# kan-bayashi/espnet

Measured on AMD Instinct MI355X. Metric: frames/sec, 12L Conformer hybrid CTC/attention training step (B=32 T=1000 d=256 per GPU), higher is better.
Workload: dtype f32; 1 GPU; BASELINE configs[1]: 12L Conformer enc d=256 h=4 ff=2048 k=31 macaron+cnn rel_pos, 6L Transformer dec, V=5000, fbank B=32 T=1000 L=100, mtlalpha 0.3, lsm 0.1; global_batch=32, frames=1000, parallelism=dp1, optimizer=adam+noam, clip 5.0, launch=hipGraph, wgrad_side_stream=False, optimizer_steps_done=113

## Files before the change

### espnet_amd/csrc/ffn_f32.hip

```cpp
#include <stdlib.h>
#include <type_traits>
#include "common.h"
#include "../../include/espnet_amd.h"
#include "ffn_ln.h"
#include "ln_bwd_rows.h"

bool eamd_ffn_bf16_ok(const eamd_ffn_t* p);
int eamd_ffn_bf16_launch(const eamd_ffn_t* p, int bwd, void* stream);

namespace {

constexpr int FBM = 32;
constexpr int FD = 256;
constexpr int FHC = 128;
constexpr int FNT = 512;
constexpr int XS_LD = 264;
constexpr int HS_LD = 136;
constexpr int XS_SZ = FBM * XS_LD;
constexpr int HS_SZ = FBM * HS_LD;

constexpr int D_SMEM_FLOATS = XS_SZ + 4 * HS_SZ;

template <bool BWD, int ACT>
__global__ __launch_bounds__(FNT, 2) void ffn_f32_direct_kernel(const eamd_ffn_t p) {
  extern __shared__ __attribute__((aligned(16))) float sm[];
  float* const xs = sm;
  float* const hs = xs + XS_SZ;
  float* const fs = hs + 2 * HS_SZ;
  const int t = threadIdx.x;
  const int lane = t & 63, wave = __builtin_amdgcn_readfirstlane(t >> 6);
  const bool up = wave < 4;
  const int wq = wave & 3;
  const int fr = lane & 15, fq = lane >> 4;
  const int m0 = blockIdx.x * FBM;
  const int F = p.F;
  const int nch = F / FHC / (int)gridDim.y;
  const int hid0 = (int)blockIdx.y * nch * FHC;
  const int nsteps = 8 * nch;
  const bool full_rows = m0 + FBM <= p.M;
  using T_ = std::true_type;
  using F_ = std::false_type;

  if (!BWD && p.ln_x) {
    ffn_ln_stage(p, m0, t, [&](int row, int col, float4 y) __attribute__((always_inline)) {
      *reinterpret_cast<f32x4*>(&xs[row * XS_LD + col]) = (f32x4){y.x, y.y, y.z, y.w};
    });
  } else {
#pragma unroll
    for (int i = 0; i < 4; ++i) {
      const int idx = t + FNT * i, row = idx >> 6, c4 = idx & 63;
      *reinterpret_cast<f32x4*>(&xs[row * XS_LD + c4 * 4]) =
          *reinterpret_cast<const f32x4*>(p.x + (long)min(m0 + row, p.M - 1) * FD + c4 * 4);
    }
  }
  __syncthreads();

  if (up) {
    const float* __restrict__ W = p.w1 + (long)hid0 * FD;
    const int lc0 = wq * 32 + 2 * fr;
    constexpr int LCJ = 1;
    f32x4 bs[4][4];
    f32x4 zacc[2][2], zold[2][2];
#pragma unroll
    for (int i = 0; i < 2; ++i)
#pragma unroll
      for (int j = 0; j < 2; ++j) { zacc[i][j] = (f32x4){0.f, 0.f, 0.f, 0.f}; zold[i][j] = zacc[i][j]; }
    const unsigned thr_in = eamd_drop_thr16(p.p_in);
    const float inv_in = p.p_in > 0.f ? eamd_drop_inv(thr_in) : 1.f;
    const unsigned seed_in = (!BWD && p.p_in > 0.f) ? eamd_drop_seed((const unsigned long long*)p.drop_step, p.salt_in) : 0u;
    float bpre[2] = {0.f, 0.f};
    float fpre[2][2][4];
    const unsigned e_toff = (unsigned)(((fq * 4) * F + lc0) * 4);

    auto load_b = [&](auto set_c, int g) __attribute__((always_inline)) {
      constexpr int SET = decltype(set_c)::value;
      const char* base = reinterpret_cast<const char*>(W) + ((long)min(g, nsteps - 1) * 4 + wq) * 4096 + lane * 16;
#pragma unroll
      for (int v = 0; v < 4; ++v) bs[SET][v] = *reinterpret_cast<const f32x4*>(base + v * 1024);
    };
    float fA[2][2][4];
    auto read_a = [&](auto s_c, auto half_c) __attribute__((always_inline)) {
      constexpr int s = decltype(s_c)::value, hh = decltype(half_c)::value;
#pragma unroll
      for (int i = 0; i < 2; ++i) {
        const float4 v = *reinterpret_cast<const float4*>(&xs[(i * 16 + fr) * XS_LD + s * 32 + hh * 16 + fq * 4]);
        fA[hh][i][0] = v.x; fA[hh][i][1] = v.y; fA[hh][i][2] = v.z; fA[hh][i][3] = v.w;
      }
    };
    auto mfma_half = [&](auto set_c, auto half_c) __attribute__((always_inline)) {
      constexpr int SET = decltype(set_c)::value, q = decltype(half_c)::value;
#pragma unroll
      for (int e = 0; e < 4; ++e)
#pragma unroll
        for (int i = 0; i < 2; ++i)
#pragma unroll
          for (int j = 0; j < 2; ++j) {
            const float b = BWD ? bs[SET][q * 2 + (e >> 1)][(e & 1) * 2 + j] : bs[SET][q * 2 + j][e];
            zacc[i][j] = __builtin_amdgcn_mfma_f32_16x16x4f32(fA[q][i][e], b, zacc[i][j], 0, 0, 0);
          }
    };
    auto epi_quarter = [&](auto i_c, auto rr_c, int c) __attribute__((always_inline)) {
      constexpr int i = decltype(i_c)::value, rr = decltype(rr_c)::value;
      float* hp = hs + (c & 1) * HS_SZ;
      float* fp = fs + (c & 1) * HS_SZ;
#pragma unroll
      for (int r2 = 0; r2 < 2; ++r2) {
        constexpr int dummy = 0; (void)dummy;
        const int r = rr * 2 + r2;
// ... 14 lines not shown
          for (int j = 0; j < 2; ++j) hv[j] = (zold[i][j][r] * fpre[i][j][r]) * p.alpha;
        }
        *reinterpret_cast<float2*>(&hp[(i * 16 + fq * 4 + r) * HS_LD + lc0]) = make_float2(hv[0], hv[1]);
      }
    };
    auto load_f = [&](int c) __attribute__((always_inline)) {
      const char* base = reinterpret_cast<const char*>(p.f + (long)m0 * F + hid0 + c * FHC);
#pragma unroll
      for (int i = 0; i < 2; ++i)
#pragma unroll
        for (int r = 0; r < 4; ++r) {
          const long ro = full_rows ? (long)(i * 16 + r) * F : (long)(min(m0 + i * 16 + fq * 4 + r, p.M - 1) - m0 - fq * 4) * F;
          const float2 v = *reinterpret_cast<const float2*>(base + ro * 4 + e_toff);
          fpre[i][0][r] = v.x; fpre[i][1][r] = v.y;
        }
    };
    auto step = [&](auto s_c, auto up_c, auto epi_c, int P) __attribute__((always_inline)) {
      constexpr int s = decltype(s_c)::value;
      constexpr bool UP = decltype(up_c)::value, EPI = decltype(epi_c)::value;
      if constexpr (UP) {
        load_b(std::integral_constant<int, (s + 3) & 3>{}, 8 * P + s + 3);
        if constexpr (s == 4) {
          if constexpr (BWD) load_f(P);
          else if (p.b1) { bpre[0] = p.b1[hid0 + P * FHC + lc0]; bpre[1] = p.b1[hid0 + P * FHC + lc0 + 1]; }
        }
        __builtin_amdgcn_sched_barrier(0);
        read_a(s_c, std::integral_constant<int, 1>{});
        mfma_half(std::integral_constant<int, s & 3>{}, std::integral_constant<int, 0>{});
      }
      if constexpr (EPI && s < 4) epi_quarter(std::integral_constant<int, s & 1>{}, std::integral_constant<int, (s / 2)>{}, P - 1);
      if constexpr (UP) {
        __builtin_amdgcn_sched_barrier(0);
        read_a(std::integral_constant<int, (s + 1) & 7>{}, std::integral_constant<int, 0>{});
        mfma_half(std::integral_constant<int, s & 3>{}, std::integral_constant<int, 1>{});
        if constexpr (s == 7) {
#pragma unroll
          for (int i = 0; i < 2; ++i)
#pragma unroll
            for (int j = 0; j < 2; ++j) { zold[i][j] = zacc[i][j]; zacc[i][j] = (f32x4){0.f, 0.f, 0.f, 0.f}; }
        }
      }
      if constexpr (s == 7) __syncthreads();
    };
    auto period = [&](auto up_c, auto epi_c, int P) __attribute__((always_inline)) {
      step(std::integral_constant<int, 0>{}, up_c, epi_c, P);
      step(std::integral_constant<int, 1>{}, up_c, epi_c, P);
      step(std::integral_constant<int, 2>{}, up_c, epi_c, P);
      step(std::integral_constant<int, 3>{}, up_c, epi_c, P);
      step(std::integral_constant<int, 4>{}, up_c, epi_c, P);
      step(std::integral_constant<int, 5>{}, up_c, epi_c, P);
      step(std::integral_constant<int, 6>{}, up_c, epi_c, P);
      step(std::integral_constant<int, 7>{}, up_c, epi_c, P);
    };
    load_b(std::integral_constant<int, 0>{}, 0);
    load_b(std::integral_constant<int, 1>{}, 1);
    load_b(std::integral_constant<int, 2>{}, 2);
    read_a(std::integral_constant<int, 0>{}, std::integral_constant<int, 0>{});
    period(T_{}, F_{}, 0);
    for (int P = 1; P < nch; ++P) period(T_{}, T_{}, P);
    period(F_{}, T_{}, nch);
    period(F_{}, F_{}, nch + 1);
  } else {
    const float* __restrict__ W = p.w2 + (long)hid0 * FD;
    f32x4 bs[4][4];
    f32x4 yacc[2][4];
#pragma unroll
    for (int i = 0; i < 2; ++i)
#pragma unroll
      for (int j = 0; j < 4; ++j) yacc[i][j] = (f32x4){0.f, 0.f, 0.f, 0.f};
    auto load_b = [&](auto set_c, int gd) __attribute__((always_inline)) {
      constexpr int SET = decltype(set_c)::value;
      const char* base = reinterpret_cast<const char*>(W) + ((long)min(max(gd, 0), nsteps - 1) * 4 + wq) * 4096 + lane * 16;
#pragma unroll
      for (int v = 0; v < 4; ++v) bs[SET][v] = *reinterpret_cast<const f32x4*>(base + v * 1024);
    };
    float fA[2][2][4];
    auto read_a = [&](auto par_c, int sd, int hbuf) __attribute__((always_inline)) {
      constexpr int PAR = decltype(par_c)::value;
      const float* hp = hs + hbuf * HS_SZ;
#pragma unroll
      for (int i = 0; i < 2; ++i) {
        const float4 v = *reinterpret_cast<const float4*>(&hp[(i * 16 + fr) * HS_LD + sd * 16 + fq * 4]);
        fA[PAR][i][0] = v.x; fA[PAR][i][1] = v.y; fA[PAR][i][2] = v.z; fA[PAR][i][3] = v.w;
      }
    };
    auto mfma_step = [&](auto set_c, auto par_c) __attribute__((always_inline)) {
      constexpr int SET = decltype(set_c)::value, PAR = decltype(par_c)::value;
#pragma unroll
      for (int e = 0; e < 4; ++e)
#pragma unroll
        for (int i = 0; i < 2; ++i)
#pragma unroll
          for (int j = 0; j < 4; ++j) {
            const float b = BWD ? bs[SET][e][j] : bs[SET][j][e];
            yacc[i][j] = __builtin_amdgcn_mfma_f32_16x16x4f32(fA[PAR][i][e], b, yacc[i][j], 0, 0, 0);
          }
    };
    auto step = [&](auto s_c, auto d_c, auto dn_c, int P) __attribute__((always_inline)) {
      constexpr int s = decltype(s_c)::value;
      constexpr bool D = decltype(d_c)::value, DN = decltype(dn_c)::value;
      const int gd = 8 * (P - 2) + s;
      if constexpr (s + 3 < 8 ? D : DN) load_b(std::integral_constant<int, (s + 3) & 3>{}, gd + 3);
      if constexpr (D && (s == 1 || s == 3)) {
        float* dstp = (s == 1) ? p.h : (BWD ? nullptr : p.f);
        if (dstp) {
          const float* src = (s == 1 ? hs : fs) + (P & 1) * HS_SZ;
          const int dt = t - 256;
#pragma unroll
          for (int k = 0; k < 4; ++k) {
            const int idx = dt + 256 * k, lr = idx >> 5, c4 = idx & 31;
            if (full_rows || m0 + lr < p.M)
              *reinterpret_cast<float4*>(dstp + (long)(m0 + lr) * F + hid0 + (P - 2) * FHC + c4 * 4) =
                  *reinterpret_cast<const float4*>(&src[lr * HS_LD + c4 * 4]);
          }
        }
      }
      if constexpr (D) {
        __builtin_amdgcn_sched_barrier(0);
        if constexpr (s < 7) read_a(std::integral_constant<int, (s + 1) & 1>{}, s + 1, P & 1);
        mfma_step(std::integral_constant<int, s & 3>{}, std::integral_constant<int, s & 1>{});
      }
      if constexpr (s == 7) {
        __syncthreads();
        if constexpr (DN) read_a(std::integral_constant<int, 0>{}, 0, (P + 1) & 1);
      }
    };
    auto period = [&](auto d_c, auto dn_c, int P) __attribute__((always_inline)) {
      step(std::integral_constant<int, 0>{}, d_c, dn_c, P);
      step(std::integral_constant<int, 1>{}, d_c, dn_c, P);
      step(std::integral_constant<int, 2>{}, d_c, dn_c, P);
      step(std::integral_constant<int, 3>{}, d_c, dn_c, P);
      step(std::integral_constant<int, 4>{}, d_c, dn_c, P);
      step(std::integral_constant<int, 5>{}, d_c, dn_c, P);
      step(std::integral_constant<int, 6>{}, d_c, dn_c, P);
      step(std::integral_constant<int, 7>{}, d_c, dn_c, P);
    };
    period(F_{}, F_{}, 0);
    period(F_{}, T_{}, 1);
    for (int P = 2; P <= nch; ++P) period(T_{}, T_{}, P);
    period(T_{}, F_{}, nch + 1);
#pragma unroll
    for (int i = 0; i < 2; ++i)
#pragma unroll
      for (int r = 0; r < 4; ++r) {
        if constexpr (BWD) {
          *reinterpret_cast<float4*>(&xs[(i * 16 + fq * 4 + r) * XS_LD + wq * 64 + 4 * fr]) =
              make_float4(yacc[i][0][r], yacc[i][1][r], yacc[i][2][r], yacc[i][3][r]);
        } else {
#pragma unroll
          for (int j = 0; j < 4; ++j) xs[(i * 16 + fq * 4 + r) * XS_LD + wq * 64 + j * 16 + fr] = yacc[i][j][r];
        }
      }
  }
  __syncthreads();
  if constexpr (BWD) {
    if (p.lnb_x) {
      const EamdLnbArgs la{p.lnb_x, p.lnb_gamma, p.lnb_mean, p.lnb_rstd, p.lnb_dres, p.lnb_ws, p.lnb_drop_out, p.lnb_drop_p,
                           (unsigned long long)p.lnb_drop_salt, p.drop_step, p.out, (long)FD, p.M};
      eamd_ln_bwd_rows32<XS_LD>(la, xs, hs, hs + FBM * FD, m0, t, (int)blockIdx.x);
      return;
    }
  }
  const unsigned thr_out = eamd_drop_thr16(p.p_out);
  const float inv_out = eamd_drop_inv(thr_out);
  const unsigned seed_out = (!BWD && p.p_out > 0.f) ? eamd_drop_seed((const unsigned long long*)p.drop_step, p.salt_out) : 0u;
#pragma unroll
  for (int i = 0; i < 4; ++i) {
    const int idx = t + FNT * i, lr = idx >> 6, c4 = idx & 63;
    const int row = m0 + lr;
    if (row >= p.M) continue;
    const float4 a4 = *reinterpret_cast<const float4*>(&xs[lr * XS_LD + c4 * 4]);
    float v[4] = {a4.x, a4.y, a4.z, a4.w};
    const long gi = (long)row * FD + c4 * 4;
    const bool first = blockIdx.y == 0;
    if constexpr (!BWD) {
      if (p.b2 && first) {
        const float4 b4 = *reinterpret_cast<const float4*>(p.b2 + c4 * 4);
        v[0] += b4.x; v[1] += b4.y; v[2] += b4.z; v[3] += b4.w;
      }
      if (p.p_out > 0.f) {
        bool keep[4];
        eamd_drop_keep4(seed_out, (unsigned long long)gi, thr_out, keep);
#pragma unroll
        for (int e = 0; e < 4; ++e) v[e] = keep[e] ? v[e] * inv_out : 0.f;
      }
      float4 r4 = make_float4(0.f, 0.f, 0.f, 0.f);
      if (p.R && first) r4 = *reinterpret_cast<const float4*>(p.R + gi);
      v[0] = v[0] * p.alpha + r4.x; v[1] = v[1] * p.alpha + r4.y; v[2] = v[2] * p.alpha + r4.z; v[3] = v[3] * p.alpha + r4.w;
    }
    if (gridDim.y > 1) {
#pragma unroll
      for (int e = 0; e < 4; ++e) atomicAdd(p.out + gi + e, v[e]);
    } else {
      *reinterpret_cast<float4*>(p.out + gi) = make_float4(v[0], v[1], v[2], v[3]);
    }
  }
}

__global__ __launch_bounds__(256) void ffn_pack_f32_kernel(const float* __restrict__ w1, const float* __restrict__ w2,
                                                           float* __restrict__ p0, float* __restrict__ p1,
                                                           float* __restrict__ p2, float* __restrict__ p3, int F) {
  const int which = blockIdx.y;
  const long piece = (long)blockIdx.x * 256 + threadIdx.x;
  const long npiece = (long)(F / FHC) * 8 * 4 * 4 * 64;
  if (piece >= npiece) return;
  const int lane = piece & 63, v = (piece >> 6) & 3, wq = (piece >> 8) & 3;
  const int g = (int)(piece >> 10), c = g >> 3, s = g & 7;
  const int fr = lane & 15, fq = lane >> 4;
  float4 o;
  if (which == 0) {
    const int q = v >> 1, j = v & 1;
    o = *reinterpret_cast<const float4*>(w1 + (long)(c * FHC + wq * 32 + 2 * fr + j) * FD + s * 32 + q * 16 + fq * 4);
    *reinterpret_cast<float4*>(p0 + piece * 4) = o;
  } else if (which == 1) {
    o = *reinterpret_cast<const float4*>(w2 + (long)(wq * 64 + v * 16 + fr) * F + c * FHC + s * 16 + fq * 4);
    *reinterpret_cast<float4*>(p1 + piece * 4) = o;
  } else if (which == 2) {
    const int q = v >> 1, e0 = (v & 1) * 2;
    const float* r0 = w2 + (long)(s * 32 + q * 16 + fq * 4 + e0) * F + c * FHC + wq * 32 + 2 * fr;
    const float2 a = *reinterpret_cast<const float2*>(r0), b = *reinterpret_cast<const float2*>(r0 + F);
    *reinterpret_cast<float4*>(p2 + piece * 4) = make_float4(a.x, a.y, b.x, b.y);
  } else {
    o = *reinterpret_cast<const float4*>(w1 + (long)(c * FHC + s * 16 + fq * 4 + v) * FD + wq * 64 + 4 * fr);
    *reinterpret_cast<float4*>(p3 + piece * 4) = o;
  }
}

constexpr int FFN_PACK_JOBS = 32;
struct FfnPackJob { const float* w1; const float* w2; float* p0; float* p1; float* p2; float* p3; int F; int pad; };
struct FfnPackTable { FfnPackJob j[FFN_PACK_JOBS]; };
__global__ __launch_bounds__(256) void ffn_pack_f32_multi_kernel(const FfnPackTable tab) {
  const FfnPackJob jb = tab.j[blockIdx.z];
  const int which = blockIdx.y, F = jb.F;
  const long npiece = (long)(F / FHC) * 8 * 4 * 4 * 64;
  for (long piece = (long)blockIdx.x * 256 + threadIdx.x; piece < npiece; piece += (long)gridDim.x * 256) {
    const int lane = piece & 63, v = (piece >> 6) & 3, wq = (piece >> 8) & 3;
    const int g = (int)(piece >> 10), c = g >> 3, s = g & 7;
    const int fr = lane & 15, fq = lane >> 4;
    if (which == 0) {
      const int q = v >> 1, j = v & 1;
// ... 126 lines not shown
```

### espnet_amd/csrc/ffn_ln.h

```cpp
#pragma once
#include "common.h"
#include "../../include/espnet_amd.h"

template <typename Put>
__device__ __forceinline__ void ffn_ln_stage(const eamd_ffn_t& p, const int m0, const int t, Put&& put) {
  constexpr int D = 256;
  const int row = t >> 4, l = t & 15;
  const bool live = m0 + row < p.M;
  const long gr = (long)min(m0 + row, p.M - 1);
  const float4* __restrict__ xr = reinterpret_cast<const float4*>(p.ln_x + gr * D);
  float4 v[4];
  float s = 0.f;
#pragma unroll
  for (int j = 0; j < 4; ++j) { v[j] = xr[l + 16 * j]; s += v[j].x + v[j].y + v[j].z + v[j].w; }
#pragma unroll
  for (int m = 1; m < 16; m <<= 1) s += __shfl_xor(s, m);
  const float mean = s / D;
  float q = 0.f;
#pragma unroll
  for (int j = 0; j < 4; ++j) {
    const float a = v[j].x - mean, b = v[j].y - mean, c = v[j].z - mean, d = v[j].w - mean;
    q += a * a + b * b + c * c + d * d;
  }
#pragma unroll
  for (int m = 1; m < 16; m <<= 1) q += __shfl_xor(q, m);
  const float rstd = rsqrtf(q / D + p.ln_eps);
  const float4* __restrict__ g4 = reinterpret_cast<const float4*>(p.ln_w);
  const float4* __restrict__ b4 = reinterpret_cast<const float4*>(p.ln_b);
#pragma unroll
  for (int j = 0; j < 4; ++j) {
    const float4 g = g4[l + 16 * j], b = b4[l + 16 * j];
    float4 o;
    o.x = (v[j].x - mean) * rstd * g.x + b.x;
    o.y = (v[j].y - mean) * rstd * g.y + b.y;
    o.z = (v[j].z - mean) * rstd * g.z + b.z;
    o.w = (v[j].w - mean) * rstd * g.w + b.w;
    const int col = (l + 16 * j) * 4;
    put(row, col, o);
    if (live) {
      if (p.dtype == 1) {
        uint2 h;
        h.x = eamd_f2bf(o.x) | ((unsigned)eamd_f2bf(o.y) << 16);
        h.y = eamd_f2bf(o.z) | ((unsigned)eamd_f2bf(o.w) << 16);
        *reinterpret_cast<uint2*>(reinterpret_cast<unsigned short*>(const_cast<float*>(p.x)) + gr * D + col) = h;
      } else {
        *reinterpret_cast<float4*>(const_cast<float*>(p.x) + gr * D + col) = o;
      }
    }
  }
  if (live && l == 0) { p.ln_mean[gr] = mean; p.ln_rstd[gr] = rstd; }
}
```

### espnet_amd/csrc/ln_bwd_rows.h

```cpp
#pragma once
#include "common.h"

struct EamdLnbArgs {
  const float* x; const float* gamma; const float* mean; const float* rstd; const float* dres;
  float* ws; float* drop_out; float drop_p; unsigned long long drop_salt; const void* drop_step;
  float* out; long ldo; int M;
};

template <int TLD>
__device__ __forceinline__ void eamd_ln_bwd_rows32(const EamdLnbArgs& a, const float* tile, float* gs, float* bsum, const int m0,
                                                   const int t, const int blk) {
  constexpr int D = 256;
  const int row = t >> 4, l = t & 15;
  const bool live = m0 + row < a.M;
  const long gr = (long)min(m0 + row, a.M - 1);
  const float mu = a.mean[gr], rs = a.rstd[gr];
  float4 dq[4], h4[4], g4[4], rv[4];
  float s1 = 0.f, s2 = 0.f;
#pragma unroll
  for (int j = 0; j < 4; ++j) {
    const int col = (l + 16 * j) * 4;
    dq[j] = *reinterpret_cast<const float4*>(&tile[row * TLD + col]);
    const float4 xv = *reinterpret_cast<const float4*>(a.x + gr * D + col);
    g4[j] = *reinterpret_cast<const float4*>(a.gamma + col);
    rv[j] = a.dres ? *reinterpret_cast<const float4*>(a.dres + gr * D + col) : make_float4(0.f, 0.f, 0.f, 0.f);
    h4[j] = make_float4((xv.x - mu) * rs, (xv.y - mu) * rs, (xv.z - mu) * rs, (xv.w - mu) * rs);
    const float p0 = dq[j].x * g4[j].x, p1 = dq[j].y * g4[j].y, p2 = dq[j].z * g4[j].z, p3 = dq[j].w * g4[j].w;
    s1 += (p0 + p1) + (p2 + p3);
    s2 += (p0 * h4[j].x + p1 * h4[j].y) + (p2 * h4[j].z + p3 * h4[j].w);
  }
#pragma unroll
  for (int m = 1; m < 16; m <<= 1) { s1 += __shfl_xor(s1, m); s2 += __shfl_xor(s2, m); }
  s1 /= D; s2 /= D;
  const unsigned thr_d = eamd_drop_thr16(a.drop_p);
  const float inv_d = eamd_drop_inv(thr_d);
  const unsigned seed_d = a.drop_out ? eamd_drop_seed((const unsigned long long*)a.drop_step, a.drop_salt) : 0u;
  const float z = live ? 1.f : 0.f;
#pragma unroll
  for (int j = 0; j < 4; ++j) {
    const int col = (l + 16 * j) * 4;
    float4 o;
    o.x = rs * (dq[j].x * g4[j].x - s1 - h4[j].x * s2) + rv[j].x;
    o.y = rs * (dq[j].y * g4[j].y - s1 - h4[j].y * s2) + rv[j].y;
    o.z = rs * (dq[j].z * g4[j].z - s1 - h4[j].z * s2) + rv[j].z;
    o.w = rs * (dq[j].w * g4[j].w - s1 - h4[j].w * s2) + rv[j].w;
    if (live) {
      *reinterpret_cast<float4*>(a.out + gr * a.ldo + col) = o;
      if (a.drop_out) {
        bool keep[4];
        eamd_drop_keep4(seed_d, (unsigned long long)(gr * D + col), thr_d, keep);
        *reinterpret_cast<float4*>(a.drop_out + gr * D + col) =
            make_float4(keep[0] ? o.x * inv_d : 0.f, keep[1] ? o.y * inv_d : 0.f, keep[2] ? o.z * inv_d : 0.f,
                        keep[3] ? o.w * inv_d : 0.f);
      }
    }
    *reinterpret_cast<float4*>(&gs[row * D + col]) =
        make_float4(z * dq[j].x * h4[j].x, z * dq[j].y * h4[j].y, z * dq[j].z * h4[j].z, z * dq[j].w * h4[j].w);
    *reinterpret_cast<float4*>(&bsum[row * D + col]) = make_float4(z * dq[j].x, z * dq[j].y, z * dq[j].z, z * dq[j].w);
  }
  __syncthreads();
  const float* src = (t < D ? gs : bsum) + (t & (D - 1));
  float s = 0.f;
#pragma unroll 8
  for (int r = 0; r < 32; ++r) s += src[r * D];
  a.ws[(long)blk * 2 * D + t] = s;
}
```

### espnet_amd/csrc/rowproj_f32.hip

```cpp
#include <stdlib.h>
#include <type_traits>
#include "common.h"
#include "../../include/espnet_amd.h"
#include "ln_bwd_rows.h"

namespace {

constexpr int RBM = 32;
constexpr int RNT = 512;
constexpr int RCH = 256;
constexpr int ST_LD = 36;
constexpr int ST_SZ = RBM * ST_LD;
constexpr int TL_LD = 264;

__device__ __forceinline__ int xs_ld(int K) { return K + 8; }

__device__ __forceinline__ void stage_ln(const eamd_rowproj_t& p, const int m0, const int t, float* xs, const int LD) {
  constexpr int D = 256;
  const int row = t >> 4, l = t & 15;
  const bool live = m0 + row < p.M;
  const long gr = (long)min(m0 + row, p.M - 1);
  const float4* __restrict__ xr = reinterpret_cast<const float4*>(p.ln_x + gr * D);
  float4 v[4];
  float s = 0.f;
#pragma unroll
  for (int j = 0; j < 4; ++j) { v[j] = xr[l + 16 * j]; s += v[j].x + v[j].y + v[j].z + v[j].w; }
#pragma unroll
  for (int m = 1; m < 16; m <<= 1) s += __shfl_xor(s, m);
  const float mean = s / D;
  float q = 0.f;
#pragma unroll
  for (int j = 0; j < 4; ++j) {
    const float a = v[j].x - mean, b = v[j].y - mean, c = v[j].z - mean, d = v[j].w - mean;
    q += a * a + b * b + c * c + d * d;
  }
#pragma unroll
  for (int m = 1; m < 16; m <<= 1) q += __shfl_xor(q, m);
  const float rstd = rsqrtf(q / D + p.ln_eps);
  const float4* __restrict__ g4 = reinterpret_cast<const float4*>(p.ln_w);
  const float4* __restrict__ b4 = reinterpret_cast<const float4*>(p.ln_b);
#pragma unroll
  for (int j = 0; j < 4; ++j) {
    const float4 g = g4[l + 16 * j], b = b4[l + 16 * j];
    float4 o;
    o.x = (v[j].x - mean) * rstd * g.x + b.x;
    o.y = (v[j].y - mean) * rstd * g.y + b.y;
    o.z = (v[j].z - mean) * rstd * g.z + b.z;
    o.w = (v[j].w - mean) * rstd * g.w + b.w;
    const int col = (l + 16 * j) * 4;
    *reinterpret_cast<float4*>(&xs[row * LD + col]) = o;
    if (live) *reinterpret_cast<float4*>(const_cast<float*>(p.a) + gr * D + col) = o;
  }
  if (live && l == 0) { p.ln_mean[gr] = mean; p.ln_rstd[gr] = rstd; }
}

__device__ __forceinline__ void stage_affine(const eamd_rowproj_t& p, const int m0, const int t, float* xs, const int LD) {
  constexpr int D = 256;
#pragma unroll
  for (int i = 0; i < 4; ++i) {
    const int idx = t + RNT * i, row = idx >> 6, c4 = idx & 63;
    const long gr = (long)min(m0 + row, p.M - 1);
    const float4 v = *reinterpret_cast<const float4*>(p.a + gr * p.lda + c4 * 4);
    const float4 sc = *reinterpret_cast<const float4*>(p.a_scale + c4 * 4), sh = *reinterpret_cast<const float4*>(p.a_shift + c4 * 4);
    float4 o;
    o.x = eamd_act(v.x * sc.x + sh.x, p.a_act); o.y = eamd_act(v.y * sc.y + sh.y, p.a_act);
    o.z = eamd_act(v.z * sc.z + sh.z, p.a_act); o.w = eamd_act(v.w * sc.w + sh.w, p.a_act);
    *reinterpret_cast<float4*>(&xs[row * LD + c4 * 4]) = o;
    if (p.a_out && m0 + row < p.M) *reinterpret_cast<float4*>(p.a_out + gr * D + c4 * 4) = o;
  }
}

template <bool LNB>
__global__ __launch_bounds__(RNT, 2) void rowproj_f32_kernel(const eamd_rowproj_t p) {
  extern __shared__ __attribute__((aligned(16))) float sm[];
  const int K = p.K, N = p.N;
  const int LD = xs_ld(K);
  float* const xs = sm;
  const int t = threadIdx.x;
  const int lane = t & 63, wave = __builtin_amdgcn_readfirstlane(t >> 6);
  const int fr = lane & 15, fq = lane >> 4;
  const int m0 = blockIdx.x * RBM;
  const int S = K >> 5;
  const int nchunk = N / RCH;
  const int nsteps = S * nchunk;
  float* const st = sm + RBM * LD + wave * ST_SZ;

  if (p.ln_x) {
    stage_ln(p, m0, t, xs, LD);
  } else if (p.a_scale) {
    stage_affine(p, m0, t, xs, LD);
  } else {
    const int c4n = K >> 2;
    for (int idx = t; idx < RBM * c4n; idx += RNT) {
      const int row = idx / c4n, c4 = idx - row * c4n;
      *reinterpret_cast<f32x4*>(&xs[row * LD + c4 * 4]) =
          *reinterpret_cast<const f32x4*>(p.a + (long)min(m0 + row, p.M - 1) * p.lda + c4 * 4);
    }
  }

  const char* __restrict__ Wb = reinterpret_cast<const char*>(p.w) + (long)wave * 4096 + lane * 16;
  f32x4 bs[4][4];
  auto load_b = [&](auto set_c, int g) __attribute__((always_inline)) {
    constexpr int SET = decltype(set_c)::value;
    const char* base = Wb + (long)min(g, nsteps - 1) * (8 * 4096);
#pragma unroll
    for (int v = 0; v < 4; ++v) bs[SET][v] = *reinterpret_cast<const f32x4*>(base + v * 1024);
  };
  float fA[2][2][4];
  auto read_a = [&](int kcol, auto half_c) __attribute__((always_inline)) {
    constexpr int hh = decltype(half_c)::value;
#pragma unroll
    for (int i = 0; i < 2; ++i) {
      const float4 v = *reinterpret_cast<const float4*>(&xs[(i * 16 + fr) * LD + kcol + hh * 16 + fq * 4]);
      fA[hh][i][0] = v.x; fA[hh][i][1] = v.y; fA[hh][i][2] = v.z; fA[hh][i][3] = v.w;
    }
  };
  f32x4 acc[2][2];
  auto mfma_half = [&](auto set_c, auto half_c) __attribute__((always_inline)) {
    constexpr int SET = decltype(set_c)::value, q = decltype(half_c)::value;
#pragma unroll
    for (int e = 0; e < 4; ++e)
#pragma unroll
      for (int i = 0; i < 2; ++i)
#pragma unroll
        for (int j = 0; j < 2; ++j)
          acc[i][j] = __builtin_amdgcn_mfma_f32_16x16x4f32(fA[q][i][e], bs[SET][q * 2 + j][e], acc[i][j], 0, 0, 0);
  };
  using I0 = std::integral_constant<int, 0>;
  using I1 = std::integral_constant<int, 1>;
  auto step = [&](auto s_c, int g, int kcol, int kcol_next) __attribute__((always_inline)) {
    constexpr int s = decltype(s_c)::value;
    load_b(std::integral_constant<int, (s + 3) & 3>{}, g + 3);
    __builtin_amdgcn_sched_barrier(0);
    read_a(kcol, I1{});
    mfma_half(std::integral_constant<int, s & 3>{}, I0{});
    __builtin_amdgcn_sched_barrier(0);
    read_a(kcol_next, I0{});
    mfma_half(std::integral_constant<int, s & 3>{}, I1{});
  };

  load_b(std::integral_constant<int, 0>{}, 0);
  load_b(std::integral_constant<int, 1>{}, 1);
  load_b(std::integral_constant<int, 2>{}, 2);
  __syncthreads();
  read_a(0, I0{});

  const unsigned thr_out = eamd_drop_thr16(p.p_out);
  const float inv_out = eamd_drop_inv(thr_out);
  const unsigned seed_out = p.p_out > 0.f ? eamd_drop_seed((const unsigned long long*)p.drop_step, p.salt_out) : 0u;

  int g = 0;
  for (int c = 0; c < nchunk; ++c) {
#pragma unroll
    for (int i = 0; i < 2; ++i)
#pragma unroll
      for (int j = 0; j < 2; ++j) acc[i][j] = (f32x4){0.f, 0.f, 0.f, 0.f};
    for (int kp = 0; kp < S; kp += 4) {
      const int k0 = kp * 32;
      step(std::integral_constant<int, 0>{}, g + 0, k0, k0 + 32);
      step(std::integral_constant<int, 1>{}, g + 1, k0 + 32, k0 + 64);
      step(std::integral_constant<int, 2>{}, g + 2, k0 + 64, k0 + 96);
      step(std::integral_constant<int, 3>{}, g + 3, k0 + 96, (kp + 4 < S) ? k0 + 128 : 0);
      g += 4;
    }
    if constexpr (!LNB) {
#pragma unroll
      for (int i = 0; i < 2; ++i)
#pragma unroll
        for (int r = 0; r < 4; ++r)
          *reinterpret_cast<float2*>(&st[(i * 16 + fq * 4 + r) * ST_LD + 2 * fr]) = make_float2(acc[i][0][r], acc[i][1][r]);
      __builtin_amdgcn_fence(__ATOMIC_RELEASE, "wavefront");
      __builtin_amdgcn_wave_barrier();
      __builtin_amdgcn_fence(__ATOMIC_ACQUIRE, "wavefront");
      const int col0 = c * RCH + wave * 32 + (lane & 7) * 4;
      float4 b4 = make_float4(0.f, 0.f, 0.f, 0.f);
      if (p.bias) b4 = *reinterpret_cast<const float4*>(p.bias + col0);
#pragma unroll
      for (int it = 0; it < 4; ++it) {
        const int lr = it * 8 + (lane >> 3);
        const int row = m0 + lr;
        const float4 a4 = *reinterpret_cast<const float4*>(&st[lr * ST_LD + (lane & 7) * 4]);
        if (row < p.M) {
          float v[4] = {a4.x + b4.x, a4.y + b4.y, a4.z + b4.z, a4.w + b4.w};
          const long gi = (long)row * N + col0;
          if (p.p_out > 0.f) {
            bool keep[4];
            eamd_drop_keep4(seed_out, (unsigned long long)gi, thr_out, keep);
#pragma unroll
            for (int e = 0; e < 4; ++e) v[e] = keep[e] ? v[e] * inv_out : 0.f;
          }
          float4 r4 = make_float4(0.f, 0.f, 0.f, 0.f);
          if (p.R) r4 = *reinterpret_cast<const float4*>(p.R + (long)row * p.ldr + col0);
          *reinterpret_cast<float4*>(p.out + (long)row * p.ldo + col0) =
              make_float4(v[0] * p.alpha + r4.x, v[1] * p.alpha + r4.y, v[2] * p.alpha + r4.z, v[3] * p.alpha + r4.w);
        }
      }
      __builtin_amdgcn_wave_barrier();
    }
  }

  if constexpr (LNB) {
    constexpr int D = 256;
    float* const tl = sm;
    float* const gs = sm + RBM * TL_LD;
    float* const bsum = gs + RBM * D;
    __syncthreads();
#pragma unroll
    for (int i = 0; i < 2; ++i)
#pragma unroll
      for (int r = 0; r < 4; ++r)
        *reinterpret_cast<float2*>(&tl[(i * 16 + fq * 4 + r) * TL_LD + wave * 32 + 2 * fr]) = make_float2(acc[i][0][r], acc[i][1][r]);
    __syncthreads();
    const EamdLnbArgs la{p.lnb_x, p.lnb_gamma, p.lnb_mean, p.lnb_rstd, p.lnb_dres, p.lnb_ws, p.lnb_drop_out, p.lnb_drop_p,
                         (unsigned long long)p.lnb_drop_salt, p.drop_step, p.out, (long)p.ldo, p.M};
    eamd_ln_bwd_rows32<TL_LD>(la, tl, gs, bsum, m0, t, (int)blockIdx.x);
  }
}

struct PackJob { const float* w; float* img; int K, N, ldw, trans; long npiece; };
constexpr int PACK_JOBS = 48;
struct PackTable { PackJob j[PACK_JOBS]; };
__global__ __launch_bounds__(256) void rowproj_pack_kernel(const PackTable tab) {
  const PackJob jb = tab.j[blockIdx.y];
  for (long piece = (long)blockIdx.x * 256 + threadIdx.x; piece < jb.npiece; piece += (long)gridDim.x * 256) {
    const int lane = piece & 63, v = (piece >> 6) & 3, w = (piece >> 8) & 7;
    const long gs_ = piece >> 11;
    const int S = jb.K >> 5;
    const int c = (int)(gs_ / S), s = (int)(gs_ - (long)c * S);
    const int fr = lane & 15, fq = lane >> 4, q = v >> 1, j = v & 1;
    const int col = c * RCH + w * 32 + 2 * fr + j, k = s * 32 + q * 16 + fq * 4;
    float4 o;
    if (jb.trans) {
      const float* r0 = jb.w + (long)k * jb.ldw + col;
      o = make_float4(r0[0], r0[jb.ldw], r0[2L * jb.ldw], r0[3L * jb.ldw]);
    } else {
      o = *reinterpret_cast<const float4*>(jb.w + (long)col * jb.ldw + k);
    }
    *reinterpret_cast<float4*>(jb.img + piece * 4) = o;
  }
}

bool al16(const void* q) { return (reinterpret_cast<uintptr_t>(q) & 15) == 0; }

size_t smem_bytes(int K, bool lnb) {
  size_t rows = (size_t)RBM * (K + 8);
  if (lnb) {
    const size_t need = (size_t)RBM * TL_LD + 2 * (size_t)RBM * 256;
    return (rows > need ? rows : need) * sizeof(float);
  }
  return (rows + 8 * (size_t)ST_SZ) * sizeof(float);
}

int check_rowproj(const eamd_rowproj_t* p) {
  if (!p || !p->a || !p->w || !p->out) return EAMD_EINVAL;
  if (p->M <= 0 || p->K <= 0 || p->N <= 0) return EAMD_EINVAL;
  if (p->K % 256 != 0 || p->N % RCH != 0 || p->K > 768) return EAMD_EUNSUPPORTED;
  if (p->lda < p->K || p->ldo < p->N || (p->R && p->ldr < p->N)) return EAMD_EINVAL;
  if (p->lda % 4 != 0 || p->ldo % 4 != 0 || (p->R && p->ldr % 4 != 0)) return EAMD_EUNSUPPORTED;
  if (!al16(p->a) || !al16(p->w) || !al16(p->out) || (p->R && !al16(p->R)) || (p->bias && !al16(p->bias))) return EAMD_EUNSUPPORTED;
  if (p->p_out < 0.f || p->p_out >= 1.f) return EAMD_EINVAL;
  if (p->p_out > 0.f && (!p->drop_step || p->ldo != p->N)) return EAMD_EINVAL;
  if (p->ln_x) {
    if (p->K != 256 || p->a_scale || !p->ln_w || !p->ln_b || !p->ln_mean || !p->ln_rstd || p->lda != 256) return EAMD_EINVAL;
    if (!al16(p->ln_x) || !al16(p->ln_w) || !al16(p->ln_b)) return EAMD_EUNSUPPORTED;
  }
  if (p->a_scale) {
    if (p->K != 256 || !p->a_shift) return EAMD_EINVAL;
    if (!al16(p->a_scale) || !al16(p->a_shift) || (p->a_out && !al16(p->a_out))) return EAMD_EUNSUPPORTED;
// ... 57 lines not shown
```

Baseline: 1.147 million frames/s.

## Prefetch epilogue operands and overlap weight loads with row staging in FFN/rowproj kernels

The first weight-tile loads are now issued while activation rows are being staged, whether through LN, affine or a plain copy, instead of after staging finishes. Epilogue operands (residual, bias, and the LN-backward x/dres/gamma/mean/rstd) are prefetched into registers during the last MFMA steps rather than loaded after the GEMM. The goal is to hide global-memory latency at kernel start and in the epilogue. In exchange it raises register pressure, which may hurt occupancy at launch_bounds(512,2), and the rowproj K-loop is restructured to peel its last group.

```diff
diff --git a/espnet_amd/csrc/ffn_f32.hip b/espnet_amd/csrc/ffn_f32.hip
--- a/espnet_amd/csrc/ffn_f32.hip
+++ b/espnet_amd/csrc/ffn_f32.hip
@@ -41,19 +41,56 @@
   using T_ = std::true_type;
   using F_ = std::false_type;
 
-  if (!BWD && p.ln_x) {
-    ffn_ln_stage(p, m0, t, [&](int row, int col, float4 y) __attribute__((always_inline)) {
-      *reinterpret_cast<f32x4*>(&xs[row * XS_LD + col]) = (f32x4){y.x, y.y, y.z, y.w};
-    });
-  } else {
-#pragma unroll
-    for (int i = 0; i < 4; ++i) {
-      const int idx = t + FNT * i, row = idx >> 6, c4 = idx & 63;
-      *reinterpret_cast<f32x4*>(&xs[row * XS_LD + c4 * 4]) =
-          *reinterpret_cast<const f32x4*>(p.x + (long)min(m0 + row, p.M - 1) * FD + c4 * 4);
-    }
-  }
-  __syncthreads();
+  auto stage_rows = [&](auto&& issue_w) __attribute__((always_inline)) {
+    if (!BWD && p.ln_x) {
+      ffn_ln_stage(p, m0, t, [&](int row, int col, float4 y) __attribute__((always_inline)) {
+        *reinterpret_cast<f32x4*>(&xs[row * XS_LD + col]) = (f32x4){y.x, y.y, y.z, y.w};
+      }, issue_w);
+    } else {
+      f32x4 v[4];
+#pragma unroll
+      for (int i = 0; i < 4; ++i) {
+        const int idx = t + FNT * i, row = idx >> 6, c4 = idx & 63;
+        v[i] = *reinterpret_cast<const f32x4*>(p.x + (long)min(m0 + row, p.M - 1) * FD + c4 * 4);
+      }
+      issue_w();
+#pragma unroll
+      for (int i = 0; i < 4; ++i) {
+        const int idx = t + FNT * i, row = idx >> 6, c4 = idx & 63;
+        *reinterpret_cast<f32x4*>(&xs[row * XS_LD + c4 * 4]) = v[i];
+      }
+    }
+    __syncthreads();
+  };
+
+  const bool first = blockIdx.y == 0;
+  const EamdLnbArgs la{p.lnb_x, p.lnb_gamma, p.lnb_mean, p.lnb_rstd, p.lnb_dres, p.lnb_ws, p.lnb_drop_out, p.lnb_drop_p,
+                       (unsigned long long)p.lnb_drop_salt, p.drop_step, p.out, (long)FD, p.M};
+  EamdLnbPre pre;
+  float4 b2p = make_float4(0.f, 0.f, 0.f, 0.f), rp[4];
+  auto epi_pre = [&](auto part_c) __attribute__((always_inline)) {
+    constexpr int part = decltype(part_c)::value;
+    if constexpr (BWD) {
+      if (p.lnb_x) {
+        if constexpr (part == 0) eamd_ln_bwd_prefetch_x(la, pre, m0, t);
+        if constexpr (part == 1) eamd_ln_bwd_prefetch_dres(la, pre, m0, t);
+        if constexpr (part == 2) eamd_ln_bwd_prefetch_gamma(la, pre, t);
+      }
+    } else {
+      if constexpr (part == 0) {
+#pragma unroll
+        for (int i = 0; i < 4; ++i) rp[i] = make_float4(0.f, 0.f, 0.f, 0.f);
+        if (p.R && first) {
+#pragma unroll
+          for (int i = 0; i < 4; ++i)
+            rp[i] = *reinterpret_cast<const float4*>(p.R + (long)min(m0 + ((t + FNT * i) >> 6), p.M - 1) * FD + (t & 63) * 4);
+        }
+      }
+      if constexpr (part == 1) {
+        if (p.b2 && first) b2p = *reinterpret_cast<const float4*>(p.b2 + (t & 63) * 4);
+      }
+    }
+  };
 
   if (up) {
     const float* __restrict__ W = p.w1 + (long)hid0 * FD;
@@ -174,13 +211,18 @@
       step(std::integral_constant<int, 6>{}, up_c, epi_c, P);
       step(std::integral_constant<int, 7>{}, up_c, epi_c, P);
     };
-    load_b(std::integral_constant<int, 0>{}, 0);
-    load_b(std::integral_constant<int, 1>{}, 1);
-    load_b(std::integral_constant<int, 2>{}, 2);
+    stage_rows([&]() __attribute__((always_inline)) {
+      load_b(std::integral_constant<int, 0>{}, 0);
+      load_b(std::integral_constant<int, 1>{}, 1);
+      load_b(std::integral_constant<int, 2>{}, 2);
+    });
     read_a(std::integral_constant<int, 0>{}, std::integral_constant<int, 0>{});
     period(T_{}, F_{}, 0);
     for (int P = 1; P < nch; ++P) period(T_{}, T_{}, P);
     period(F_{}, T_{}, nch);
+    epi_pre(std::integral_constant<int, 0>{});
+    epi_pre(std::integral_constant<int, 1>{});
+    epi_pre(std::integral_constant<int, 2>{});
     period(F_{}, F_{}, nch + 1);
   } else {
     const float* __restrict__ W = p.w2 + (long)hid0 * FD;
@@ -223,6 +265,7 @@
       constexpr bool D = decltype(d_c)::value, DN = decltype(dn_c)::value;
       const int gd = 8 * (P - 2) + s;
       if constexpr (s + 3 < 8 ? D : DN) load_b(std::integral_constant<int, (s + 3) & 3>{}, gd + 3);
+      if constexpr (D && !DN && s >= 5) epi_pre(std::integral_constant<int, s - 5>{});
       if constexpr (D && (s == 1 || s == 3)) {
         float* dstp = (s == 1) ? p.h : (BWD ? nullptr : p.f);
         if (dstp) {
@@ -257,6 +300,7 @@
       step(std::integral_constant<int, 6>{}, d_c, dn_c, P);
       step(std::integral_constant<int, 7>{}, d_c, dn_c, P);
     };
+    stage_rows([]() {});
     period(F_{}, F_{}, 0);
     period(F_{}, T_{}, 1);
     for (int P = 2; P <= nch; ++P) period(T_{}, T_{}, P);
@@ -277,9 +321,7 @@
   __syncthreads();
   if constexpr (BWD) {
     if (p.lnb_x) {
-      const EamdLnbArgs la{p.lnb_x, p.lnb_gamma, p.lnb_mean, p.lnb_rstd, p.lnb_dres, p.lnb_ws, p.lnb_drop_out, p.lnb_drop_p,
-                           (unsigned long long)p.lnb_drop_salt, p.drop_step, p.out, (long)FD, p.M};
-      eamd_ln_bwd_rows32<XS_LD>(la, xs, hs, hs + FBM * FD, m0, t, (int)blockIdx.x);
+      eamd_ln_bwd_rows32<XS_LD>(la, pre, xs, hs, hs + FBM * FD, m0, t, (int)blockIdx.x);
       return;
     }
   }
@@ -294,10 +336,9 @@
     const float4 a4 = *reinterpret_cast<const float4*>(&xs[lr * XS_LD + c4 * 4]);
     float v[4] = {a4.x, a4.y, a4.z, a4.w};
     const long gi = (long)row * FD + c4 * 4;
-    const bool first = blockIdx.y == 0;
     if constexpr (!BWD) {
       if (p.b2 && first) {
-        const float4 b4 = *reinterpret_cast<const float4*>(p.b2 + c4 * 4);
+        const float4 b4 = b2p;
         v[0] += b4.x; v[1] += b4.y; v[2] += b4.z; v[3] += b4.w;
       }
       if (p.p_out > 0.f) {
@@ -306,8 +347,7 @@
 #pragma unroll
         for (int e = 0; e < 4; ++e) v[e] = keep[e] ? v[e] * inv_out : 0.f;
       }
-      float4 r4 = make_float4(0.f, 0.f, 0.f, 0.f);
-      if (p.R && first) r4 = *reinterpret_cast<const float4*>(p.R + gi);
+      const float4 r4 = rp[i];
       v[0] = v[0] * p.alpha + r4.x; v[1] = v[1] * p.alpha + r4.y; v[2] = v[2] * p.alpha + r4.z; v[3] = v[3] * p.alpha + r4.w;
     }
     if (gridDim.y > 1) {
diff --git a/espnet_amd/csrc/ffn_ln.h b/espnet_amd/csrc/ffn_ln.h
--- a/espnet_amd/csrc/ffn_ln.h
+++ b/espnet_amd/csrc/ffn_ln.h
@@ -2,17 +2,24 @@
 #include "common.h"
 #include "../../include/espnet_amd.h"
 
-template <typename Put>
-__device__ __forceinline__ void ffn_ln_stage(const eamd_ffn_t& p, const int m0, const int t, Put&& put) {
+template <typename Put, typename Issue>
+__device__ __forceinline__ void ffn_ln_stage(const eamd_ffn_t& p, const int m0, const int t, Put&& put, Issue&& issue_w) {
   constexpr int D = 256;
   const int row = t >> 4, l = t & 15;
   const bool live = m0 + row < p.M;
   const long gr = (long)min(m0 + row, p.M - 1);
   const float4* __restrict__ xr = reinterpret_cast<const float4*>(p.ln_x + gr * D);
-  float4 v[4];
+  const float4* __restrict__ g4 = reinterpret_cast<const float4*>(p.ln_w);
+  const float4* __restrict__ b4 = reinterpret_cast<const float4*>(p.ln_b);
+  float4 v[4], gv[4], bv[4];
+#pragma unroll
+  for (int j = 0; j < 4; ++j) v[j] = xr[l + 16 * j];
+#pragma unroll
+  for (int j = 0; j < 4; ++j) { gv[j] = g4[l + 16 * j]; bv[j] = b4[l + 16 * j]; }
+  issue_w();
   float s = 0.f;
 #pragma unroll
-  for (int j = 0; j < 4; ++j) { v[j] = xr[l + 16 * j]; s += v[j].x + v[j].y + v[j].z + v[j].w; }
+  for (int j = 0; j < 4; ++j) s += v[j].x + v[j].y + v[j].z + v[j].w;
 #pragma unroll
   for (int m = 1; m < 16; m <<= 1) s += __shfl_xor(s, m);
   const float mean = s / D;
@@ -25,11 +32,9 @@
 #pragma unroll
   for (int m = 1; m < 16; m <<= 1) q += __shfl_xor(q, m);
   const float rstd = rsqrtf(q / D + p.ln_eps);
-  const float4* __restrict__ g4 = reinterpret_cast<const float4*>(p.ln_w);
-  const float4* __restrict__ b4 = reinterpret_cast<const float4*>(p.ln_b);
 #pragma unroll
   for (int j = 0; j < 4; ++j) {
-    const float4 g = g4[l + 16 * j], b = b4[l + 16 * j];
+    const float4 g = gv[j], b = bv[j];
     float4 o;
     o.x = (v[j].x - mean) * rstd * g.x + b.x;
     o.y = (v[j].y - mean) * rstd * g.y + b.y;
@@ -50,3 +55,8 @@
   }
   if (live && l == 0) { p.ln_mean[gr] = mean; p.ln_rstd[gr] = rstd; }
 }
+
+template <typename Put>
+__device__ __forceinline__ void ffn_ln_stage(const eamd_ffn_t& p, const int m0, const int t, Put&& put) {
+  ffn_ln_stage(p, m0, t, put, []() {});
+}
diff --git a/espnet_amd/csrc/ln_bwd_rows.h b/espnet_amd/csrc/ln_bwd_rows.h
--- a/espnet_amd/csrc/ln_bwd_rows.h
+++ b/espnet_amd/csrc/ln_bwd_rows.h
@@ -7,23 +7,47 @@
   float* out; long ldo; int M;
 };
 
+struct EamdLnbPre { float mu, rs; float4 xv[4], g4[4], rv[4]; };
+
+__device__ __forceinline__ void eamd_ln_bwd_prefetch_x(const EamdLnbArgs& a, EamdLnbPre& pre, const int m0, const int t) {
+  constexpr int D = 256;
+  const int row = t >> 4, l = t & 15;
+  const long gr = (long)min(m0 + row, a.M - 1);
+  pre.mu = a.mean[gr]; pre.rs = a.rstd[gr];
+#pragma unroll
+  for (int j = 0; j < 4; ++j) pre.xv[j] = *reinterpret_cast<const float4*>(a.x + gr * D + (l + 16 * j) * 4);
+}
+__device__ __forceinline__ void eamd_ln_bwd_prefetch_dres(const EamdLnbArgs& a, EamdLnbPre& pre, const int m0, const int t) {
+  constexpr int D = 256;
+  const int row = t >> 4, l = t & 15;
+  const long gr = (long)min(m0 + row, a.M - 1);
+#pragma unroll
+  for (int j = 0; j < 4; ++j)
+    pre.rv[j] = a.dres ? *reinterpret_cast<const float4*>(a.dres + gr * D + (l + 16 * j) * 4) : make_float4(0.f, 0.f, 0.f, 0.f);
+}
+__device__ __forceinline__ void eamd_ln_bwd_prefetch_gamma(const EamdLnbArgs& a, EamdLnbPre& pre, const int t) {
+  const int l = t & 15;
+#pragma unroll
+  for (int j = 0; j < 4; ++j) pre.g4[j] = *reinterpret_cast<const float4*>(a.gamma + (l + 16 * j) * 4);
+}
+
 template <int TLD>
-__device__ __forceinline__ void eamd_ln_bwd_rows32(const EamdLnbArgs& a, const float* tile, float* gs, float* bsum, const int m0,
-                                                   const int t, const int blk) {
+__device__ __forceinline__ void eamd_ln_bwd_rows32(const EamdLnbArgs& a, const EamdLnbPre& pre, const float* tile, float* gs,
+                                                   float* bsum, const int m0, const int t, const int blk) {
   constexpr int D = 256;
   const int row = t >> 4, l = t & 15;
   const bool live = m0 + row < a.M;
   const long gr = (long)min(m0 + row, a.M - 1);
-  const float mu = a.mean[gr], rs = a.rstd[gr];
+  const float mu = pre.mu, rs = pre.rs;
   float4 dq[4], h4[4], g4[4], rv[4];
   float s1 = 0.f, s2 = 0.f;
 #pragma unroll
   for (int j = 0; j < 4; ++j) {
     const int col = (l + 16 * j) * 4;
     dq[j] = *reinterpret_cast<const float4*>(&tile[row * TLD + col]);
-    const float4 xv = *reinterpret_cast<const float4*>(a.x + gr * D + col);
-    g4[j] = *reinterpret_cast<const float4*>(a.gamma + col);
-    rv[j] = a.dres ? *reinterpret_cast<const float4*>(a.dres + gr * D + col) : make_float4(0.f, 0.f, 0.f, 0.f);
+    const float4 xv = pre.xv[j];
+    g4[j] = pre.g4[j];
+    rv[j] = pre.rv[j];
     h4[j] = make_float4((xv.x - mu) * rs, (xv.y - mu) * rs, (xv.z - mu) * rs, (xv.w - mu) * rs);
     const float p0 = dq[j].x * g4[j].x, p1 = dq[j].y * g4[j].y, p2 = dq[j].z * g4[j].z, p3 = dq[j].w * g4[j].w;
     s1 += (p0 + p1) + (p2 + p3);
diff --git a/espnet_amd/csrc/rowproj_f32.hip b/espnet_amd/csrc/rowproj_f32.hip
--- a/espnet_amd/csrc/rowproj_f32.hip
+++ b/espnet_amd/csrc/rowproj_f32.hip
@@ -15,16 +15,24 @@
 
 __device__ __forceinline__ int xs_ld(int K) { return K + 8; }
 
-__device__ __forceinline__ void stage_ln(const eamd_rowproj_t& p, const int m0, const int t, float* xs, const int LD) {
+template <typename Issue>
+__device__ __forceinline__ void stage_ln(const eamd_rowproj_t& p, const int m0, const int t, float* xs, const int LD, Issue&& issue_w) {
   constexpr int D = 256;
   const int row = t >> 4, l = t & 15;
   const bool live = m0 + row < p.M;
   const long gr = (long)min(m0 + row, p.M - 1);
   const float4* __restrict__ xr = reinterpret_cast<const float4*>(p.ln_x + gr * D);
-  float4 v[4];
+  const float4* __restrict__ g4 = reinterpret_cast<const float4*>(p.ln_w);
+  const float4* __restrict__ b4 = reinterpret_cast<const float4*>(p.ln_b);
+  float4 v[4], gv[4], bv[4];
+#pragma unroll
+  for (int j = 0; j < 4; ++j) v[j] = xr[l + 16 * j];
+#pragma unroll
+  for (int j = 0; j < 4; ++j) { gv[j] = g4[l + 16 * j]; bv[j] = b4[l + 16 * j]; }
+  issue_w();
   float s = 0.f;
 #pragma unroll
-  for (int j = 0; j < 4; ++j) { v[j] = xr[l + 16 * j]; s += v[j].x + v[j].y + v[j].z + v[j].w; }
+  for (int j = 0; j < 4; ++j) s += v[j].x + v[j].y + v[j].z + v[j].w;
 #pragma unroll
   for (int m = 1; m < 16; m <<= 1) s += __shfl_xor(s, m);
   const float mean = s / D;
@@ -37,11 +45,9 @@
 #pragma unroll
   for (int m = 1; m < 16; m <<= 1) q += __shfl_xor(q, m);
   const float rstd = rsqrtf(q / D + p.ln_eps);
-  const float4* __restrict__ g4 = reinterpret_cast<const float4*>(p.ln_w);
-  const float4* __restrict__ b4 = reinterpret_cast<const float4*>(p.ln_b);
 #pragma unroll
   for (int j = 0; j < 4; ++j) {
-    const float4 g = g4[l + 16 * j], b = b4[l + 16 * j];
+    const float4 g = gv[j], b = bv[j];
     float4 o;
     o.x = (v[j].x - mean) * rstd * g.x + b.x;
     o.y = (v[j].y - mean) * rstd * g.y + b.y;
@@ -54,20 +60,54 @@
   if (live && l == 0) { p.ln_mean[gr] = mean; p.ln_rstd[gr] = rstd; }
 }
 
-__device__ __forceinline__ void stage_affine(const eamd_rowproj_t& p, const int m0, const int t, float* xs, const int LD) {
+template <typename Issue>
+__device__ __forceinline__ void stage_affine(const eamd_rowproj_t& p, const int m0, const int t, float* xs, const int LD,
+                                             Issue&& issue_w) {
   constexpr int D = 256;
+  const int c4 = t & 63;
+  float4 vv[4];
+#pragma unroll
+  for (int i = 0; i < 4; ++i)
+    vv[i] = *reinterpret_cast<const float4*>(p.a + (long)min(m0 + ((t + RNT * i) >> 6), p.M - 1) * p.lda + c4 * 4);
+  const float4 sc = *reinterpret_cast<const float4*>(p.a_scale + c4 * 4), sh = *reinterpret_cast<const float4*>(p.a_shift + c4 * 4);
+  issue_w();
 #pragma unroll
   for (int i = 0; i < 4; ++i) {
-    const int idx = t + RNT * i, row = idx >> 6, c4 = idx & 63;
+    const int row = (t + RNT * i) >> 6;
     const long gr = (long)min(m0 + row, p.M - 1);
-    const float4 v = *reinterpret_cast<const float4*>(p.a + gr * p.lda + c4 * 4);
-    const float4 sc = *reinterpret_cast<const float4*>(p.a_scale + c4 * 4), sh = *reinterpret_cast<const float4*>(p.a_shift + c4 * 4);
+    const float4 v = vv[i];
     float4 o;
     o.x = eamd_act(v.x * sc.x + sh.x, p.a_act); o.y = eamd_act(v.y * sc.y + sh.y, p.a_act);
     o.z = eamd_act(v.z * sc.z + sh.z, p.a_act); o.w = eamd_act(v.w * sc.w + sh.w, p.a_act);
     *reinterpret_cast<float4*>(&xs[row * LD + c4 * 4]) = o;
     if (p.a_out && m0 + row < p.M) *reinterpret_cast<float4*>(p.a_out + gr * D + c4 * 4) = o;
   }
+}
+
+template <typename Issue>
+__device__ __forceinline__ void stage_plain(const eamd_rowproj_t& p, const int m0, const int t, float* xs, const int LD,
+                                            Issue&& issue_w) {
+  const int c4n = p.K >> 2;
+  const int ngrp = __builtin_amdgcn_readfirstlane(p.K >> 8);
+  f32x4 v[12];
+  auto each = [&](int grp, auto&& f) __attribute__((always_inline)) {
+#pragma unroll
+    for (int i = grp * 4; i < grp * 4 + 4; ++i) {
+      const int idx = t + RNT * i, row = idx / c4n, c4 = idx - row * c4n;
+      f(i, row, c4);
+    }
+  };
+  auto ld = [&](int i, int row, int c4) __attribute__((always_inline)) {
+    v[i] = *reinterpret_cast<const f32x4*>(p.a + (long)min(m0 + row, p.M - 1) * p.lda + c4 * 4);
+  };
+  auto st = [&](int i, int row, int c4) __attribute__((always_inline)) { *reinterpret_cast<f32x4*>(&xs[row * LD + c4 * 4]) = v[i]; };
+  each(0, ld);
+  if (ngrp > 1) each(1, ld);
+  if (ngrp > 2) each(2, ld);
+  issue_w();
+  each(0, st);
+  if (ngrp > 1) each(1, st);
+  if (ngrp > 2) each(2, st);
 }
 
 template <bool LNB>
@@ -85,19 +125,6 @@
   const int nsteps = S * nchunk;
   float* const st = sm + RBM * LD + wave * ST_SZ;
 
-  if (p.ln_x) {
-    stage_ln(p, m0, t, xs, LD);
-  } else if (p.a_scale) {
-    stage_affine(p, m0, t, xs, LD);
-  } else {
-    const int c4n = K >> 2;
-    for (int idx = t; idx < RBM * c4n; idx += RNT) {
-      const int row = idx / c4n, c4 = idx - row * c4n;
-      *reinterpret_cast<f32x4*>(&xs[row * LD + c4 * 4]) =
-          *reinterpret_cast<const f32x4*>(p.a + (long)min(m0 + row, p.M - 1) * p.lda + c4 * 4);
-    }
-  }
-
   const char* __restrict__ Wb = reinterpret_cast<const char*>(p.w) + (long)wave * 4096 + lane * 16;
   f32x4 bs[4][4];
   auto load_b = [&](auto set_c, int g) __attribute__((always_inline)) {
@@ -106,6 +133,19 @@
 #pragma unroll
     for (int v = 0; v < 4; ++v) bs[SET][v] = *reinterpret_cast<const f32x4*>(base + v * 1024);
   };
+  auto first_b = [&]() __attribute__((always_inline)) {
+    load_b(std::integral_constant<int, 0>{}, 0);
+    load_b(std::integral_constant<int, 1>{}, 1);
+    load_b(std::integral_constant<int, 2>{}, 2);
+  };
+
+  if (p.ln_x) {
+    stage_ln(p, m0, t, xs, LD, first_b);
+  } else if (p.a_scale) {
+    stage_affine(p, m0, t, xs, LD, first_b);
+  } else {
+    stage_plain(p, m0, t, xs, LD, first_b);
+  }
   float fA[2][2][4];
   auto read_a = [&](int kcol, auto half_c) __attribute__((always_inline)) {
     constexpr int hh = decltype(half_c)::value;
@@ -128,9 +168,9 @@
   };
   using I0 = std::integral_constant<int, 0>;
   using I1 = std::integral_constant<int, 1>;
-  auto step = [&](auto s_c, int g, int kcol, int kcol_next) __attribute__((always_inline)) {
+  auto step = [&](auto s_c, auto ld_c, int g, int kcol, int kcol_next) __attribute__((always_inline)) {
     constexpr int s = decltype(s_c)::value;
-    load_b(std::integral_constant<int, (s + 3) & 3>{}, g + 3);
+    if constexpr (decltype(ld_c)::value) load_b(std::integral_constant<int, (s + 3) & 3>{}, g + 3);
     __builtin_amdgcn_sched_barrier(0);
     read_a(kcol, I1{});
     mfma_half(std::integral_constant<int, s & 3>{}, I0{});
@@ -139,15 +179,27 @@
     mfma_half(std::integral_constant<int, s & 3>{}, I1{});
   };
 
-  load_b(std::integral_constant<int, 0>{}, 0);
-  load_b(std::integral_constant<int, 1>{}, 1);
-  load_b(std::integral_constant<int, 2>{}, 2);
+  using T_ = std::true_type;
+  using F_ = std::false_type;
   __syncthreads();
   read_a(0, I0{});
 
   const unsigned thr_out = eamd_drop_thr16(p.p_out);
   const float inv_out = eamd_drop_inv(thr_out);
   const unsigned seed_out = p.p_out > 0.f ? eamd_drop_seed((const unsigned long long*)p.drop_step, p.salt_out) : 0u;
+  const EamdLnbArgs la{p.lnb_x, p.lnb_gamma, p.lnb_mean, p.lnb_rstd, p.lnb_dres, p.lnb_ws, p.lnb_drop_out, p.lnb_drop_p,
+                       (unsigned long long)p.lnb_drop_salt, p.drop_step, p.out, (long)p.ldo, p.M};
+  EamdLnbPre pre;
+  float4 b4p, r4p[4];
+  auto load_r = [&](int col0) __attribute__((always_inline)) {
+#pragma unroll
+    for (int it = 0; it < 4; ++it) r4p[it] = make_float4(0.f, 0.f, 0.f, 0.f);
+    if (p.R) {
+#pragma unroll
+      for (int it = 0; it < 4; ++it)
+        r4p[it] = *reinterpret_cast<const float4*>(p.R + (long)min(m0 + it * 8 + (lane >> 3), p.M - 1) * p.ldr + col0);
+    }
+  };
 
   int g = 0;
   for (int c = 0; c < nchunk; ++c) {
@@ -155,12 +207,34 @@
     for (int i = 0; i < 2; ++i)
 #pragma unroll
       for (int j = 0; j < 2; ++j) acc[i][j] = (f32x4){0.f, 0.f, 0.f, 0.f};
-    for (int kp = 0; kp < S; kp += 4) {
+    for (int kp = 0; kp < S - 4; kp += 4) {
       const int k0 = kp * 32;
-      step(std::integral_constant<int, 0>{}, g + 0, k0, k0 + 32);
-      step(std::integral_constant<int, 1>{}, g + 1, k0 + 32, k0 + 64);
-      step(std::integral_constant<int, 2>{}, g + 2, k0 + 64, k0 + 96);
-      step(std::integral_constant<int, 3>{}, g + 3, k0 + 96, (kp + 4 < S) ? k0 + 128 : 0);
+      step(std::integral_constant<int, 0>{}, T_{}, g + 0, k0, k0 + 32);
+      step(std::integral_constant<int, 1>{}, T_{}, g + 1, k0 + 32, k0 + 64);
+      step(std::integral_constant<int, 2>{}, T_{}, g + 2, k0 + 64, k0 + 96);
+      step(std::integral_constant<int, 3>{}, T_{}, g + 3, k0 + 96, k0 + 128);
+      g += 4;
+    }
+    {
+      const int k0 = (S - 4) * 32;
+      if constexpr (LNB) {
+        step(std::integral_constant<int, 0>{}, T_{}, g + 0, k0, k0 + 32);
+        eamd_ln_bwd_prefetch_x(la, pre, m0, t);
+        step(std::integral_constant<int, 1>{}, F_{}, g + 1, k0 + 32, k0 + 64);
+        eamd_ln_bwd_prefetch_dres(la, pre, m0, t);
+        step(std::integral_constant<int, 2>{}, F_{}, g + 2, k0 + 64, k0 + 96);
+        eamd_ln_bwd_prefetch_gamma(la, pre, t);
+        step(std::integral_constant<int, 3>{}, F_{}, g + 3, k0 + 96, 0);
+      } else {
+        const int col0 = c * RCH + wave * 32 + (lane & 7) * 4;
+        b4p = make_float4(0.f, 0.f, 0.f, 0.f);
+        if (p.bias) b4p = *reinterpret_cast<const float4*>(p.bias + col0);
+        load_r(col0);
+        step(std::integral_constant<int, 0>{}, T_{}, g + 0, k0, k0 + 32);
+        step(std::integral_constant<int, 1>{}, T_{}, g + 1, k0 + 32, k0 + 64);
+        step(std::integral_constant<int, 2>{}, T_{}, g + 2, k0 + 64, k0 + 96);
+        step(std::integral_constant<int, 3>{}, T_{}, g + 3, k0 + 96, 0);
+      }
       g += 4;
     }
     if constexpr (!LNB) {
@@ -169,12 +243,11 @@
 #pragma unroll
         for (int r = 0; r < 4; ++r)
           *reinterpret_cast<float2*>(&st[(i * 16 + fq * 4 + r) * ST_LD + 2 * fr]) = make_float2(acc[i][0][r], acc[i][1][r]);
+      const int col0 = c * RCH + wave * 32 + (lane & 7) * 4;
       __builtin_amdgcn_fence(__ATOMIC_RELEASE, "wavefront");
       __builtin_amdgcn_wave_barrier();
       __builtin_amdgcn_fence(__ATOMIC_ACQUIRE, "wavefront");
-      const int col0 = c * RCH + wave * 32 + (lane & 7) * 4;
-      float4 b4 = make_float4(0.f, 0.f, 0.f, 0.f);
-      if (p.bias) b4 = *reinterpret_cast<const float4*>(p.bias + col0);
+      const float4 b4 = b4p;
 #pragma unroll
       for (int it = 0; it < 4; ++it) {
         const int lr = it * 8 + (lane >> 3);
@@ -189,8 +262,7 @@
 #pragma unroll
             for (int e = 0; e < 4; ++e) v[e] = keep[e] ? v[e] * inv_out : 0.f;
           }
-          float4 r4 = make_float4(0.f, 0.f, 0.f, 0.f);
-          if (p.R) r4 = *reinterpret_cast<const float4*>(p.R + (long)row * p.ldr + col0);
+          const float4 r4 = r4p[it];
           *reinterpret_cast<float4*>(p.out + (long)row * p.ldo + col0) =
               make_float4(v[0] * p.alpha + r4.x, v[1] * p.alpha + r4.y, v[2] * p.alpha + r4.z, v[3] * p.alpha + r4.w);
         }
@@ -211,9 +283,7 @@
       for (int r = 0; r < 4; ++r)
         *reinterpret_cast<float2*>(&tl[(i * 16 + fq * 4 + r) * TL_LD + wave * 32 + 2 * fr]) = make_float2(acc[i][0][r], acc[i][1][r]);
     __syncthreads();
-    const EamdLnbArgs la{p.lnb_x, p.lnb_gamma, p.lnb_mean, p.lnb_rstd, p.lnb_dres, p.lnb_ws, p.lnb_drop_out, p.lnb_drop_p,
-                         (unsigned long long)p.lnb_drop_salt, p.drop_step, p.out, (long)p.ldo, p.M};
-    eamd_ln_bwd_rows32<TL_LD>(la, tl, gs, bsum, m0, t, (int)blockIdx.x);
+    eamd_ln_bwd_rows32<TL_LD>(la, pre, tl, gs, bsum, m0, t, (int)blockIdx.x);
   }
 }
 
```

After: 1.157 million frames/s (median of 6 runs). No clear change (+0.9%).
